# HUBioDataLab/DrugGEN

Hardware: AMD Instinct MI355X
Metric: molecules/sec GAN step (G+D fwd+bwd), N=45 graphs (higher is better)
Workload: dtype f32

## Files before the change

### druggen_amd/_lib.py

```python
from __future__ import annotations

import ctypes
import os
import threading
from ctypes import c_char_p, c_double, c_float, c_int, c_int64, c_size_t, c_void_p

import torch

_PKG = os.path.dirname(os.path.abspath(__file__))
LIB_PATH = os.environ.get("DG_LIB") or os.path.join(_PKG, "lib", "libdruggen_hip.so")

_P = c_void_p


class FFNFwdArgs(ctypes.Structure):
    _fields_ = [(n, _P) for n in ("x", "w1_packed", "b1", "w2_packed", "b2", "gamma", "beta", "y", "h", "relu_bits", "pre_ln",
                                  "mean", "rstd")] + [("R", c_int64), ("eps", c_float)]


class FFNBwdArgs(ctypes.Structure):
    _fields_ = [(n, _P) for n in ("x", "h", "relu_bits", "pre_ln", "mean", "rstd", "gamma", "w1_dgrad_packed", "w2_dgrad_packed",
                                  "dy", "dz_add", "dz", "dh", "dx", "dgamma", "dbeta", "dw1", "db1", "dw2", "db2", "workspace")] + [
        ("workspace_bytes", c_size_t), ("R", c_int64)]


SIGNATURES = {
    "dg_version": (c_int, []),
    "dg_last_error_string": (c_char_p, []),
    "dg_hidden_bytes": (c_size_t, [c_int64, c_int, c_int]),
    "dg_hidden_scale_offset": (c_size_t, [c_int64, c_int]),
    "dg_attn_core_fwd": (c_int, [_P] * 6 + [c_int, c_int, c_int, c_float, c_int, _P]),
    "dg_attn_core_bwd": (c_int, [_P] * 10 + [c_int, c_int, c_int, c_float, c_int, _P]),
    "dg_attn_core_bwd_add": (c_int, [_P] * 11 + [c_int, c_int, c_int, c_float, c_int, _P]),
    "dg_attn_core_bwd2": (c_int, [_P] * 16 + [c_int, c_int, c_int, c_float, c_int, _P]),
    "dg_attn_core_long_workspace_bytes": (c_size_t, [c_int, c_int, c_int]),
    "dg_attn_core_long_fwd": (c_int, [_P] * 6 + [c_int, c_int, c_int, c_float, c_int, _P]),
    "dg_attn_core_long_bwd": (c_int, [_P] * 12 + [c_size_t, c_int, c_int, c_int, c_float, c_int, _P]),
    "dg_attn_core_long_bwd2": (c_int, [_P] * 17 + [c_size_t, c_int, c_int, c_int, c_float, c_int, _P]),
    "dg_attn_half_packed_bytes": (c_size_t, [c_int]),
    "dg_attn_half_pack": (c_int, [_P, _P, _P, c_int, _P]),
    "dg_attn_half_fwd": (c_int, [_P] * 14 + [c_int, c_int, c_int, c_float, c_float, c_int, _P]),
    "dg_attn_half_f32_fwd": (c_int, [_P] * 17 + [c_int, c_int, c_int, c_float, c_float, _P]),
    "dg_attn_half_f32_bwd1_workspace_bytes": (c_size_t, [c_int]),
    "dg_attn_half_f32_bwd1": (c_int, [_P] * 19 + [_P, c_size_t, c_int, c_int, c_int, c_float, _P]),
    "dg_attn_half_bwd_workspace_bytes": (c_size_t, [c_int, c_int]),
    "dg_attn_half_bwd": (c_int, [_P] * 16 + [_P, c_size_t, c_int, c_int, c_int, c_float, c_int, _P]),
    "dg_ln_residual_fwd": (c_int, [_P] * 7 + [c_int64, c_int, c_float, c_int, _P]),
    "dg_ln_workspace_bytes": (c_size_t, [c_int64, c_int]),
    "dg_ln_residual_bwd": (c_int, [_P] * 9 + [_P, c_size_t, c_int64, c_int, c_int, _P]),
    "dg_ln_residual_bwd_add": (c_int, [_P] * 10 + [_P, c_size_t, c_int64, c_int, c_int, _P]),
    "dg_ln_residual_bwd2": (c_int, [_P] * 10 + [_P, c_size_t, c_int64, c_int, c_int, _P]),
    "dg_linear_wgrad_workspace_bytes": (c_size_t, [c_int64, c_int, c_int]),
    "dg_linear_wgrad": (c_int, [_P] * 5 + [_P, c_size_t, c_int64, c_int, c_int, c_int, _P]),
    "dg_row_gemm_packed_bytes": (c_size_t, [c_int, c_int, c_int]),
    "dg_row_gemm_pack": (c_int, [_P, _P, c_int, c_int, c_int, c_int, _P]),
    "dg_row_gemm_mask_words": (c_size_t, [c_int64, c_int, c_int, c_int]),
    "dg_row_gemm": (c_int, [_P] * 3 + [c_int64, c_int, c_int, _P, c_int, _P, _P, _P, _P, _P, _P, _P, _P, c_float, c_int, _P]),
    "dg_linear_wgrad3": (c_int, [_P] * 6 + [_P, c_size_t, c_int64, c_int, _P]),
    "dg_row_gemm_pack3": (c_int, [_P, _P, _P, _P, c_int, c_int, c_int, _P]),
    "dg_row_gemm_lin3": (c_int, [_P] * 5 + [c_int64, _P, _P, _P, c_int, _P]),
    "dg_row_gemm_sum3": (c_int, [_P] * 5 + [c_int64, _P, c_int, _P]),
    "dg_linear_wgrad_batch_begin": (c_int, []),
    "dg_linear_wgrad_batch_end": (c_int, [_P]),
    "dg_launch_pair_begin": (c_int, []),
    "dg_launch_pair_end": (c_int, [_P]),
    "dg_skinny_linear_fwd": (c_int, [_P] * 4 + [c_int64, c_int, c_int, c_int, _P]),
    "dg_skinny_linear_dgrad": (c_int, [_P] * 3 + [c_int64, c_int, c_int, c_int, _P]),
    "dg_skinny_linear_wgrad": (c_int, [_P] * 5 + [c_size_t, c_int64, c_int, c_int, c_int, _P]),
    "dg_embed_node_chain": (c_int, [_P] * 9 + [c_int64, c_int, c_int, _P]),
    "dg_embed_node_bwd": (c_int, [_P] * 8 + [c_int64, c_int, c_int, _P]),
    "dg_head_chain": (c_int, [_P] * 14 + [c_int64, c_int, _P]),
    "dg_head_bwd": (c_int, [_P] * 10 + [c_int64, c_int, _P]),
    "dg_head_wgrad": (c_int, [_P] * 12 + [c_int64, _P]),
    "dg_row_gemm_pack_batch": (c_int, [_P, c_int, c_int, c_int, _P]),
    "dg_row_gemm_ln_bwd_workspace_bytes": (c_size_t, [c_int]),
    "dg_row_gemm_ln_bwd": (c_int, [_P] * 3 + [c_int64, c_int] + [_P] * 7 + [_P, c_size_t, c_int, _P]),
    "dg_row_gemm_ln_bwd_in": (c_int, [_P] * 10 + [_P, c_size_t, c_int64, c_int, c_int, c_int, _P]),
    "dg_edge_ffn_ln_workspace_bytes": (c_size_t, [c_int64, c_int, c_int]),
    "dg_edge_ffn_ln_fwd": (c_int, [_P] * 13 + [c_int64, c_int, c_int, c_float, c_int, _P]),
    "dg_edge_ffn_ln_bwd": (c_int, [_P] * 20 + [_P, c_size_t, c_int64, c_int, c_int, c_int, _P]),
    "dg_edge_ffn_ln_fwd_pair": (c_int, [ctypes.POINTER(FFNFwdArgs), ctypes.POINTER(FFNFwdArgs), c_int, c_int, c_int, _P]),
    "dg_edge_ffn_ln_bwd_pair": (c_int, [ctypes.POINTER(FFNBwdArgs), ctypes.POINTER(FFNBwdArgs), c_int, c_int, c_int, _P]),
    "dg_ffn_f32_packed_bytes": (c_size_t, []),
    "dg_ffn_f32_pack": (c_int, [_P, _P, _P, _P]),
    "dg_ffn_ln_fwd_f32": (c_int, [ctypes.POINTER(FFNFwdArgs), ctypes.POINTER(FFNFwdArgs), _P]),
    "dg_ffn_bf16_padded_rows": (c_int64, [c_int64]),
    "dg_ffn_bf16_packed_bytes": (c_size_t, []),
    "dg_ffn_bf16_pack": (c_int, [_P, _P, _P, _P]),
    "dg_ffn_bf16_mask_words": (c_size_t, [c_int64]),
    "dg_ffn_bf16_workspace_bytes": (c_size_t, [c_int64]),
    "dg_ffn_ln_fwd_bf16": (c_int, [_P] * 11 + [c_int64, c_float, _P]),
    "dg_ffn_ln_bwd_bf16": (c_int, [_P] * 18 + [_P, c_size_t, c_int64, _P]),
    "dg_embed_sym_packed_floats": (c_size_t, []),
    "dg_embed_sym_workspace_bytes": (c_size_t, [c_int, c_int]),
    "dg_embed_sym_dgrad_packed_floats": (c_size_t, []),
    "dg_embed_sym_pack_dgrad": (c_int, [_P, _P, _P]),
    "dg_embed_sym_pack": (c_int, [_P, _P, _P]),
    "dg_embed_sym_fwd": (c_int, [_P] * 6 + [c_int] * 7 + [_P]),
    "dg_embed_sym_bwd": (c_int, [_P] * 12 + [_P, c_size_t] + [c_int] * 7 + [_P]),
    "dg_embed_sym_bwd_bf16_workspace_bytes": (c_size_t, [c_int, c_int]),
    "dg_embed_sym_bwd_bf16": (c_int, [_P] * 11 + [_P, c_size_t] + [c_int] * 6 + [_P]),
    "dg_embed_sym_bwd2": (c_int, [_P] * 11 + [_P, c_size_t] + [c_int] * 7 + [_P]),
    "dg_onehot_embed_workspace_bytes": (c_size_t, [c_int, c_int]),
    "dg_onehot_embed_fwd": (c_int, [_P, _P, _P, c_int, c_int, c_int, c_int, c_int, _P]),
    "dg_onehot_embed_bwd": (c_int, [_P, _P, _P, _P, c_size_t, c_int, c_int, c_int, c_int, c_int, _P]),
    "dg_densify": (c_int, [_P, _P, _P, c_int64, c_int, c_int, c_int, _P, _P, _P, _P]),
    "dg_mol_gather": (c_int, [_P, _P, _P, c_int64, _P, c_int, c_int, c_int, c_int, _P, _P, _P, _P, _P]),
    "dg_adamw_flat": (c_int, [_P, _P, _P, _P, c_int64, c_float, c_float, c_float, c_float, c_float, c_int64, _P]),
    "dg_adamw_flat_devstep": (c_int, [_P, _P, _P, _P, c_int64, c_float, c_float, c_float, c_float, c_float, _P, _P]),
    "dg_argmax_decode": (c_int, [_P, c_int64, c_int, _P, _P]),
    "dg_decode_graph": (c_int, [_P] * 3 + [c_int] * 5 + [_P] * 8 + [_P]),
    "dg_fp_pack": (c_int, [_P, c_int, c_int64, c_int, _P, _P, _P]),
    "dg_fp_tanimoto_workspace_bytes": (c_size_t, [c_int64, c_int64]),
    "dg_fp_tanimoto": (c_int, [_P, _P, c_int64, _P, _P, c_int64, c_int, c_int, _P, _P, _P, c_size_t, _P]),
    "dg_prof_enable": (c_int, [c_int]),
    "dg_prof_reset": (c_int, []),
    "dg_prof_read": (c_int, [c_int, ctypes.POINTER(c_int64), ctypes.POINTER(c_double)]),
    "dg_set_edge_rows": (c_int, [c_int64]),
    "dg_edge_rows": (c_int64, []),
}

KERNEL_IDS = {"attn_fwd": 0, "attn_bwd": 1, "attn_bwd2": 2, "ln_fwd": 3, "ln_bwd": 4, "ln_bwd2": 5, "linear_wgrad": 6, "row_gemm": 7, "embed_sym": 8, "ffn": 9, "ffn_wgrad": 10,
              "attn_half_fwd": 11, "attn_half_bwd": 12,
              "row_gemm_e128": 13, "row_gemm_e_n384": 14, "row_gemm_e_k384": 15,
              "linear_wgrad_e128": 16, "linear_wgrad_e_n384": 17, "linear_wgrad_e_k384": 18,
              "ffn_node": 19, "ffn_wgrad_node": 20, "ffn_f32": 21, "ffn_f32_node": 22}
EDGE_ROWS = 65536
_edge_rows = EDGE_ROWS


def edge_rows() -> int:
    return _edge_rows


def set_edge_rows(rows: int = 0) -> None:
# ... 104 lines not shown
```

### druggen_amd/functional/attention.py

```python
from __future__ import annotations

import contextlib
import ctypes
import threading

import torch
from torch.autograd import Function
from torch.autograd.function import once_differentiable

from .. import _lib
from ..options import options
from ._runtime import *
from .layernorm import *
from .dense import *
from .heads import *
from .ffn import *


def _attn_shapes(q, e):
    B, N, C = q.shape
    if tuple(e.shape) != (B, N, N, C):
        raise RuntimeError(f"attn_core: edge tensor {tuple(e.shape)} does not match node tensor {tuple(q.shape)}")
    return B, N, C

# ... 96 lines not shown
    @staticmethod
    def forward(ctx, q, k, v, e, ws, wo, alpha):
        B, N, C = _attn_shapes(q, e)
        ws = None if ws is None else _c(ws)
        wo = _c(wo)
        dq, dk, dv = torch.empty_like(q), torch.empty_like(q), torch.empty_like(q)
        de = torch.empty_like(e)
        _core_bwd(q, k, v, e, ws, wo, None, dq, dk, dv, de, alpha)
        ctx.save_for_backward(q, k, v, e, ws, wo)
        ctx.alpha = alpha
        return dq, dk, dv, de

    @staticmethod
    @once_differentiable
    def backward(ctx, tq, tk, tv, te):
        q, k, v, e, ws, wo = ctx.saved_tensors
        B, N, C = _attn_shapes(q, e)
        tq, tk, tv, te = _c(tq), _c(tk), _c(tv), _c(te)
        gq, gk, gv = torch.empty_like(q), torch.empty_like(q), torch.empty_like(q)
        ge = torch.empty_like(e)
        gws = torch.empty_like(e) if ws is not None else None
        gwo = torch.empty_like(q)
        _core_bwd2(q, k, v, e, ws, wo, tq, tk, tv, te, gq, gk, gv, ge, gws, gwo, ctx.alpha)
        return gq, gk, gv, ge, gws, gwo, None


def attn_core(q, k, v, e, alpha: float, need_s: bool = True):
    s, o = _AttnCore.apply(q, k, v, e, float(alpha), bool(need_s))
    return (s if need_s else None), o


def _composite_attn_block(x1, y, wq, bq, wk, bk, wv, bv, we, be, woe, boe, won, bon, g3, b3, g4, b4, alpha, eps3,
                          eps4, need_edge):
    q, k, v = linear(x1, wq, bq), linear(x1, wk, bk), linear(x1, wv, bv)
    e = linear(y, we, be)
    s, o = attn_core(q, k, v, e, alpha, need_s=need_edge)
    x2 = linear_ln(o, won, bon, x1, g3, b3, eps3)
    if not need_edge:
        return x2
    return x2, linear_ln(s, woe, boe, y, g4, b4, eps4)


def attn_half_f32_supported(yf, N: int, C: int) -> bool:
    mode = options.attn_half_f32
    return yf.is_cuda and yf.dtype == torch.float32 and C == 128 and N <= (48 if mode == "n48" else 96) and mode != "off"


def attn_half_f32_bwd1_supported(dy2f, B: int, N: int, C: int, graph: bool = False) -> bool:
    mode = options.attn_half_f32_bwd
    return (dy2f.is_cuda and dy2f.dtype == torch.float32 and C == 128 and N <= 48 and mode != "off"
            and (B >= 128 or mode == "force") and (not graph or mode != "nograph"))


class _AttnBlock(Function):

    @staticmethod
    def forward(ctx, x1, y, wq, bq, wk, bk, wv, bv, we, be, woe, boe, won, bon, g3, b3, g4, b4, alpha, eps3, eps4,
                need_edge, ppre=None, pmean=None, prstd=None, pgamma=None, pbeta=None):
        B, N, C = x1.shape
        _check_neighbours(N)
        x1f, yf = _c(x1).reshape(-1, C), _c(y).reshape(-1, C)
        adt = x1f.dtype
        pw = lambda w_, m_: packed_weight(w_, m_, adt)
        if lin3_supported(x1f, (wq, wk, wv)):
            q, k, v = lin3(x1f, (wq, wk, wv), (bq, bk, bv))
        else:
            q = row_gemm(x1f, pw(wq, 0), C, C, bias=bq)
            k = row_gemm(x1f, pw(wk, 0), C, C, bias=bk)
            v = row_gemm(x1f, pw(wv, 0), C, C, bias=bv)
        lib = _lib.load()
        keep = any(ctx.needs_input_grad)
        o = torch.empty_like(q)
        fused_edge = need_edge and attn_half_f32_supported(yf, N, C)
        if fused_edge:
            R = yf.shape[0]
            dev = yf.device
            e = torch.empty(R, C, dtype=adt, device=dev) if keep else None
            s = torch.empty(R, C, dtype=adt, device=dev) if keep else None
            y2 = torch.empty(R, C, dtype=adt, device=dev)
            pre4 = torch.empty(R, C, dtype=adt, device=dev) if keep else None
            mean4 = torch.empty(R, dtype=torch.float32, device=dev)
            rstd4 = torch.empty(R, dtype=torch.float32, device=dev)
            with _dev(q):
                _lib.check(lib.dg_attn_half_f32_fwd(_lib.ptr(yf), _lib.ptr(q), _lib.ptr(k), _lib.ptr(v), pw(we, 0).data_ptr(),
                                                    _lib.fptr(_c(be)), pw(woe, 0).data_ptr(), _lib.fptr(_c(boe)), _lib.fptr(_c(g4)),
                                                    _lib.fptr(_c(b4)), _lib.ptr(e), _lib.ptr(s), _lib.ptr(o), _lib.ptr(y2),
                                                    _lib.ptr(pre4), _lib.ptr(mean4), _lib.ptr(rstd4), B, N, C, alpha, eps4,
                                                    _lib.stream_of(q)), "dg_attn_half_f32_fwd")
            _account("attn_half_fwd", 4 * (R * C * (5 if keep else 2) + 4 * B * N * C), 4 * R * C * C,
                     floor=4 * (R * C * 2 + 4 * B * N * C))
        else:
            e = row_gemm(yf, pw(we, 0), C, C, bias=be)
            s = torch.empty_like(e) if need_edge else None
            _core_fwd(q, k, v, e, s, o, alpha, B, N, C)
        r3 = row_gemm(o, pw(won, 0), C, C, bias=bon, residual=x1f, ln=(_c(g3), _c(b3), eps3), want_pre=keep)
        x2, mean3, rstd3, pre3 = r3 if keep else (*r3, None)
        outs = [x2.view(B, N, C)]
        ctx.alias = bool(keep and in_second_order_forward() and _alias_outputs_enabled())
        aliases = ()
        if ctx.alias:
            aliases = tuple(_weight_alias(t) for t in (wq, wk, wv, we, woe, won, g3, g4))
            wq, wk, wv, we, woe, won, g3, g4 = aliases
        saved = [x1, y, wq, wk, wv, we, woe, won, g3, g4, q, k, v, e, s, o, mean3, rstd3, pre3]
        if need_edge:
            if not fused_edge:
                r4 = row_gemm(s, pw(woe, 0), C, C, bias=boe, residual=yf, ln=(_c(g4), _c(b4), eps4), want_pre=keep)
                y2, mean4, rstd4, pre4 = r4 if keep else (*r4, None)
            outs.append(y2.view(B, N, N, C))
            saved += [mean4, rstd4, pre4]
        else:
            pre4 = None
        ctx.has_prev = ppre is not None
        if ctx.has_prev:
            saved += [ppre, pmean, prstd, pgamma]
        ctx.save_for_backward(*saved)
        ctx.cfg = (alpha, eps3, eps4, need_edge, (B, N, C))
        ctx.extra = (bq, bk, bv, be, boe, bon, b3, b4)
        ctx.set_materialize_grads(False)
        return tuple(outs) + ((pre3, pre4) if need_edge else (pre3,)) + (q, k, v, e) + aliases

    @staticmethod
    def backward(ctx, dx2, *more):
        alpha, eps3, eps4, need_edge, (B, N, C) = ctx.cfg
        galias = ()
        if ctx.alias:
            more, galias = more[:-8], more[-8:]
        sv = ctx.saved_tensors
        x1, y, wq, wk, wv, we, woe, won, g3, g4, q, k, v, e, s, o, mean3, rstd3, pre3 = sv[:19]
        mean4, rstd4, pre4 = sv[19:22] if need_edge else (None, None, None)
        bq, bk, bv, be, boe, bon, b3, b4 = ctx.extra
        if need_edge:
            dy2, add3, add4, aq, ak, av, ae = more
            if dy2 is None:
                dy2 = torch.zeros_like(pre4)
        else:
            dy2 = add4 = None
            add3, aq, ak, av, ae = more
        if dx2 is None:
            dx2 = torch.zeros_like(pre3)
        wants_w = ctx.needs_input_grad[2] and not _inputs_only()
        want_aff = any(ctx.needs_input_grad[14:18]) and not _inputs_only()
        ppre = pmean = prstd = pgamma = None
        if ctx.has_prev:
            ppre, pmean, prstd, pgamma = sv[-4:]
        second_pass = any(t is not None for t in (add3, add4, aq, ak, av, ae))
        fuse_prev = bool(ctx.has_prev and not torch.is_grad_enabled() and not second_pass and ctx.needs_input_grad[1]
                         and ctx.needs_input_grad[22] and row_gemm_ln_bwd_supported(q, C)
                         and tuple(ppre.shape) == (B * N * N, C))
        outs = _AttnBlockBwd.apply(x1, y, wq, bq, wk, bk, wv, bv, we, be, woe, boe, won, bon, g3, g4,
                                   q, k, v, e, s, o, mean3, rstd3, pre3, mean4, rstd4, pre4, dx2, dy2,
                                   add3, add4, aq, ak, av, ae,
                                   alpha, need_edge, ctx.needs_input_grad[0], ctx.needs_input_grad[1], wants_w,
                                   ppre if fuse_prev else None, pmean, prstd, pgamma, want_aff,
                                   not torch.is_grad_enabled())
        (dx1, dy, dwq, dbq, dwk, dbk, dwv, dbv, dwe, dbe, dwoe, dboe, dwon, dbon, dg3, db3, dg4, db4, dzp, dgp, dbp) = outs
        if any(g is not None for g in galias):
            dwq, dwk, dwv, dwe, dwoe, dwon, dg3, dg4 = _join_alias_grads((dwq, dwk, dwv, dwe, dwoe, dwon, dg3, dg4), galias)
        if not (ctx.needs_input_grad[25] and not _inputs_only()):
            dgp = dbp = None
        return (dx1, dy, dwq, dbq, dwk, dbk, dwv, dbv, dwe, dbe, dwoe, dboe, dwon, dbon, dg3, db3, dg4, db4,
                None, None, None, None, dzp, None, None, dgp, dbp)


def _attn_bwd_launch(q, k, v, e, ws, wo, alpha, add_e=None):
    dq, dk, dv = torch.empty_like(q), torch.empty_like(q), torch.empty_like(q)
    de = torch.empty_like(e)
    _core_bwd(q, k, v, e, ws, wo, add_e, dq, dk, dv, de, alpha)
    return dq, dk, dv, de


def _attn_bwd2_launch(q, k, v, e, ws, wo, tq, tk, tv, te, alpha):
    gq, gk, gv, gwo = (torch.empty_like(q) for _ in range(4))
    ge = torch.empty_like(e)
    gws = torch.empty_like(e) if ws is not None else None
    _core_bwd2(q, k, v, e, ws, wo, tq, tk, tv, te, gq, gk, gv, ge, gws, gwo, alpha)
    return gq, gk, gv, ge, gws, gwo


class _AttnBlockBwd(Function):

    @staticmethod
    def forward(ctx, *args):
        wants_w = args[40] or (len(args) > 45 and args[45])
        with _reduce_batch(args[0], on=bool(wants_w)) as inb:
            return _AttnBlockBwd._forward(ctx, inb, *args)

    @staticmethod
    def _forward(ctx, inb, x1, y, wq, bq, wk, bk, wv, bv, we, be, woe, boe, won, bon, g3, g4, q, k, v, e, s, o,
                 mean3, rstd3, pre3, mean4, rstd4, pre4, dx2, dy2, add3, add4, aq, ak, av, ae,
                 alpha, need_edge, want_x, want_y, wants_w, ppre=None, pmean=None, prstd=None, pgamma=None, want_aff=None,
                 no_graph=False):
        if want_aff is None:
            want_aff = wants_w
        B, N, C = x1.shape
        adt = q.dtype
        pw = lambda w_, m_: packed_weight(w_, m_, adt)
        cast = lambda t: t if t.dtype == adt else t.to(adt)
        x1f, yf = _c(x1).reshape(-1, C), _c(y).reshape(-1, C)
        dx2f = _c(cast(dx2)).reshape(-1, C)
        cadd = lambda t: None if t is None else _c(cast(t)).reshape(-1, C)
        dz3, dg3, db3 = _ln_bwd_rows(pre3, g3, mean3, rstd3, dx2f, cadd(add3), want_affine=want_aff,
                                     batch_slot=0 if inb else None)
# ... 297 lines not shown
```

### druggen_amd/options.py

```python
from __future__ import annotations

import contextlib
import os

_CHOICES = {
    "hidden": ("dh16", "dh24", "f32", "f24", "f16"),
    "ffn_f32": ("unfused", "fused"),
    "attn_half_f32": ("fused", "n48", "off"),
    "attn_half_f32_bwd": ("fused", "nograph", "off", "force"),
    "attn_half": ("fused", "unfused", "force"),
    "ffn_bf16": ("fused", "unfused"),
    "low_memory_share": ("auto", "on", "off"),
    "ln_bwd_epilogue": (True, False),
    "ln_bwd_prologue": (True, False),
    "ffn_pair": (True, False),
    "penalty_wgrad": ("joined", "engine"),
    "embed_bf16": ("fast", "general"),
}
_ENV = {"hidden": "DG_HIDDEN", "ffn_f32": "DG_FFN_F32", "attn_half_f32": "DG_ATTN_HALF_F32",
        "attn_half_f32_bwd": "DG_ATTN_HALF_F32_BWD", "attn_half": "DG_ATTN_HALF", "ffn_bf16": "DG_FFN_BF16",
        "low_memory_share": "DG_LOW_MEMORY_SHARE"}


class _Options:
    def __init__(self):
        for name, choices in _CHOICES.items():
            value = choices[0]
            env = _ENV.get(name)
            if env and os.environ.get(env) is not None:
                value = os.environ[env]
                if value not in choices:
                    raise ValueError(f"{env}={value!r}: expected one of {choices}")
            object.__setattr__(self, name, value)

    def __setattr__(self, name, value):
        if name not in _CHOICES:
            raise AttributeError(f"druggen_amd.options has no option {name!r}")
        if value not in _CHOICES[name]:
            raise ValueError(f"options.{name} = {value!r}: expected one of {_CHOICES[name]}")
        object.__setattr__(self, name, value)

    def set(self, **kw):
        for k, v in kw.items():
            setattr(self, k, v)

    @contextlib.contextmanager
    def override(self, **kw):
        prev = {k: getattr(self, k) for k in kw}
        self.set(**kw)
        try:
            yield self
        finally:
            self.set(**prev)

    def as_dict(self):
        return {k: getattr(self, k) for k in _CHOICES}


options = _Options()
```

### include/druggen_hip.h

```cpp
#ifndef DRUGGEN_HIP_H
#define DRUGGEN_HIP_H

#include <stddef.h>
#include <stdint.h>

#ifdef __cplusplus
extern "C" {
#endif

#define DG_VERSION 232
#define DG_DTYPE_F32  0
#define DG_DTYPE_BF16 1
#define DG_DTYPE_F32_H16 2
#define DG_DTYPE_F32_H24 3
#define DG_DTYPE_F32_DH16 4
#define DG_DTYPE_F32_DH24 5
#define DG_DTYPE_F32_H32 6
#define DG_DTYPE_F32_H32_DH16 7
#define DG_E_SHAPE   (-1)
#define DG_E_ARG     (-2)
#define DG_E_WORKSPACE (-3)
#define DG_EDGE_ROWS 65536

typedef void* dg_stream_t;
// ... 99 lines not shown
int dg_row_gemm_pack_batch(const void* table, int n, int max_dim, int dtype, dg_stream_t stream);
int dg_row_gemm_pack3(const float* w0, const float* w1, const float* w2, void* packed, int cols, int mode, int dtype,
                      dg_stream_t stream);
int dg_row_gemm_lin3(const void* a, const void* packed, void* y0, void* y1, void* y2, int64_t R, const float* b0,
                     const float* b1, const float* b2, int dtype, dg_stream_t stream);
int dg_row_gemm_sum3(const void* a0, const void* a1, const void* a2, const void* packed, void* y, int64_t R,
                     const void* residual, int dtype, dg_stream_t stream);
size_t dg_row_gemm_mask_words(int64_t R, int K, int N, int dtype);
int dg_row_gemm(const void* a, const void* packed, void* y, int64_t R, int K, int N,
                const float* bias, int relu, unsigned* relu_bits_out, const unsigned* mask_bits,
                const void* residual,
                const float* gamma, const float* beta, float* mean, float* rstd, void* pre_ln,
                float eps, int dtype, dg_stream_t stream);
size_t dg_row_gemm_ln_bwd_workspace_bytes(int dtype);
int dg_row_gemm_ln_bwd(const void* a, const void* packed, void* dz, int64_t R, int K, const void* residual,
                       const void* ln_pre, const float* ln_mean, const float* ln_rstd, const float* ln_gamma,
                       float* dgamma, float* dbeta, void* workspace, size_t workspace_bytes, int dtype,
                       dg_stream_t stream);
int dg_row_gemm_ln_bwd_in(const void* dy, const void* ln_pre, const float* ln_mean, const float* ln_rstd,
                          const float* ln_gamma, const void* packed, void* dz, void* y, float* dgamma, float* dbeta,
                          void* workspace, size_t workspace_bytes, int64_t R, int K, int N, int dtype,
                          dg_stream_t stream);

size_t dg_edge_ffn_ln_workspace_bytes(int64_t R, int C, int H);
int dg_edge_ffn_ln_fwd(const void* x, const void* w1_packed, const float* b1, const void* w2_packed,
                       const float* b2, const float* gamma, const float* beta,
                       void* y, void* h, unsigned* relu_bits, void* pre_ln, float* mean, float* rstd,
                       int64_t R, int C, int H, float eps, int dtype, dg_stream_t stream);
int dg_edge_ffn_ln_bwd(const void* x, const void* h, const unsigned* relu_bits, const void* pre_ln,
                       const float* mean, const float* rstd, const float* gamma,
                       const void* w1_dgrad_packed, const void* w2_dgrad_packed, const void* dy,
                       const void* dz_add,
                       void* dz, void* dh, void* dx, float* dgamma, float* dbeta,
                       float* dw1, float* db1, float* dw2, float* db2,
                       void* workspace, size_t workspace_bytes, int64_t R, int C, int H, int dtype,
                       dg_stream_t stream);

typedef struct dg_ffn_fwd_args {
    const void* x; const void* w1_packed; const float* b1; const void* w2_packed; const float* b2;
    const float* gamma; const float* beta;
    void* y; void* h; unsigned* relu_bits; void* pre_ln; float* mean; float* rstd;
    int64_t R; float eps;
} dg_ffn_fwd_args;
typedef struct dg_ffn_bwd_args {
    const void* x; const void* h; const unsigned* relu_bits; const void* pre_ln; const float* mean; const float* rstd;
    const float* gamma; const void* w1_dgrad_packed; const void* w2_dgrad_packed; const void* dy; const void* dz_add;
    void* dz; void* dh; void* dx; float* dgamma; float* dbeta; float* dw1; float* db1; float* dw2; float* db2;
    void* workspace; size_t workspace_bytes; int64_t R;
} dg_ffn_bwd_args;
int dg_edge_ffn_ln_fwd_pair(const dg_ffn_fwd_args* node, const dg_ffn_fwd_args* edge, int C, int H, int dtype,
                            dg_stream_t stream);
int dg_edge_ffn_ln_bwd_pair(const dg_ffn_bwd_args* node, const dg_ffn_bwd_args* edge, int C, int H, int dtype,
                            dg_stream_t stream);

int64_t dg_ffn_bf16_padded_rows(int64_t R);
size_t dg_ffn_bf16_packed_bytes(void);
int dg_ffn_bf16_pack(const float* w1, const float* w2, void* packed, dg_stream_t stream);
size_t dg_ffn_bf16_mask_words(int64_t R);
size_t dg_ffn_bf16_workspace_bytes(int64_t R);
int dg_ffn_ln_fwd_bf16(const void* x, const void* packed, const float* b1, const float* b2, const float* gamma,
                       const float* beta, void* y, void* pre_ln, float* mean, float* rstd, unsigned* relu_bits,
                       int64_t R, float eps, dg_stream_t stream);
int dg_ffn_ln_bwd_bf16(const void* x, const void* pre_ln, const float* mean, const float* rstd,
                       const unsigned* relu_bits, const float* gamma, const void* packed, const float* b1,
                       const void* dy, void* dz, void* dx, float* dgamma, float* dbeta,
                       float* dw1, float* db1, float* dw2, float* db2, unsigned* bits_scratch,
                       void* workspace, size_t workspace_bytes, int64_t R, dg_stream_t stream);


size_t dg_ffn_f32_packed_bytes(void);
int dg_ffn_f32_pack(const float* w1, const float* w2, void* packed, dg_stream_t stream);
int dg_ffn_ln_fwd_f32(const dg_ffn_fwd_args* node, const dg_ffn_fwd_args* edge, dg_stream_t stream);

size_t dg_embed_sym_packed_floats(void);
size_t dg_embed_sym_workspace_bytes(int B, int N);
int dg_embed_sym_pack(const float* w2, float* packed, dg_stream_t stream);
size_t dg_embed_sym_dgrad_packed_floats(void);
int dg_embed_sym_pack_dgrad(const float* w2, float* packed, dg_stream_t stream);
int dg_embed_sym_fwd(const float* a, const float* w1, const float* b1, const float* w2_packed, const float* b2,
                     void* out, int B, int N, int E, int H, int C, int act, int dtype, dg_stream_t stream);
int dg_embed_sym_bwd(const float* a, const float* w1, const float* b1, const float* w2_packed,
                     const float* w2_dgrad_packed, const float* b2, const void* g,
                     float* da, float* dw1, float* db1, float* dw2, float* db2,
                     void* workspace, size_t workspace_bytes,
                     int B, int N, int E, int H, int C, int act, int dtype, dg_stream_t stream);
size_t dg_embed_sym_bwd_bf16_workspace_bytes(int B, int N);
int dg_embed_sym_bwd_bf16(const float* a, const float* w1, const float* b1, const float* w2, const float* b2,
                          const void* g, float* da, float* dw1, float* db1, float* dw2, float* db2,
                          void* workspace, size_t workspace_bytes, int B, int N, int E, int H, int C, int act,
                          dg_stream_t stream);

int dg_embed_sym_bwd2(const float* a, const float* w1, const float* b1, const float* w2_packed,
                      const float* w2_dgrad_packed, const float* b2, const void* g, const float* t,
                      void* gg, float* gw1, float* gw2, void* workspace, size_t workspace_bytes,
                      int B, int N, int E, int H, int C, int act, int dtype, dg_stream_t stream);

size_t dg_onehot_embed_workspace_bytes(int E, int C);
int dg_onehot_embed_fwd(const int* labels, const float* table, void* out, int B, int N, int E, int C, int dtype,
                        dg_stream_t stream);
int dg_onehot_embed_bwd(const int* labels, const void* g, float* dtable, void* workspace, size_t workspace_bytes,
                        int B, int N, int E, int C, int dtype, dg_stream_t stream);

int dg_densify(const int64_t* edge_src, const int64_t* edge_dst, const int64_t* edge_attr, int64_t n_edges,
               int B, int N, int E, int* labels, float* a, int* bad_count, dg_stream_t stream);

int dg_mol_gather(const uint8_t* atoms, const int64_t* ptr, const uint32_t* entries, int64_t n, const int64_t* index, int B,
// ... 84 lines not shown
```

Measured before the change: 4862.

## Run attention block forward and backward as single native sequenced entry points

Adds dg_attn_block_fwd/bwd C entry points that issue the whole attention block's kernel sequence (qkv projection, edge projection and attention, output projections with LayerNorm, and the full backward including weight gradients) from one ctypes call. It also carves all intermediate buffers from a single allocation and bypasses the nested autograd backward Function. The aim is to cut Python dispatch, per-op ctypes overhead and allocator calls in a launch-bound small-graph workload. It is enabled by default through a new option, at the cost of a second code path that must stay consistent with the existing one.

```diff
diff --git a/druggen_amd/_lib.py b/druggen_amd/_lib.py
--- a/druggen_amd/_lib.py
+++ b/druggen_amd/_lib.py
@@ -3,7 +3,7 @@
 import ctypes
 import os
 import threading
-from ctypes import c_char_p, c_double, c_float, c_int, c_int64, c_size_t, c_void_p
+from ctypes import c_char_p, c_double, c_float, c_int, c_int64, c_size_t, c_uint, c_void_p
 
 import torch
 
@@ -22,6 +22,25 @@
     _fields_ = [(n, _P) for n in ("x", "h", "relu_bits", "pre_ln", "mean", "rstd", "gamma", "w1_dgrad_packed", "w2_dgrad_packed",
                                   "dy", "dz_add", "dz", "dh", "dx", "dgamma", "dbeta", "dw1", "db1", "dw2", "db2", "workspace")] + [
         ("workspace_bytes", c_size_t), ("R", c_int64)]
+
+
+class AttnBlockFwdArgs(ctypes.Structure):
+    _fields_ = [(n, _P) for n in ("x1", "y", "wqkv_packed", "bq", "bk", "bv", "we_packed", "be", "woe_packed", "boe", "won_packed",
+                                  "bon", "g3", "b3", "g4", "b4", "q", "k", "v", "o", "e", "s", "x2", "mean3", "rstd3", "pre3",
+                                  "y2", "mean4", "rstd4", "pre4")] + [
+        ("B", c_int), ("N", c_int), ("C", c_int), ("alpha", c_float), ("eps3", c_float), ("eps4", c_float), ("flags", c_uint)]
+
+
+class AttnBlockBwdArgs(ctypes.Structure):
+    _fields_ = [(n, _P) for n in ("x1", "y", "q", "k", "v", "e", "s", "o", "mean3", "rstd3", "pre3", "mean4", "rstd4", "pre4", "g3",
+                                  "g4", "won_dgrad_packed", "woe_dgrad_packed", "we_dgrad_packed", "wqkv_dgrad_packed", "dx2",
+                                  "dy2", "ppre", "pmean", "prstd", "pgamma", "dz3", "d_o", "dz4", "ds", "de", "dq", "dk", "dv",
+                                  "dx1", "dy", "dzp", "dgp", "dbp", "dg3", "db3", "dg4", "db4", "dwqkv", "dbqkv", "dwe", "dbe",
+                                  "dwon", "dbon", "dwoe", "dboe", "workspace")] + [
+        ("workspace_bytes", c_size_t), ("B", c_int), ("N", c_int), ("C", c_int), ("alpha", c_float), ("flags", c_uint)]
+
+
+AB_NEED_EDGE, AB_WGRAD, AB_AFFINE, AB_INPUTS_ONLY, AB_REDUCE_BATCH, AB_BWD1_FUSED, AB_LN4_IN_GEMM = 1, 2, 4, 8, 16, 32, 64
 
 
 SIGNATURES = {
@@ -81,6 +100,9 @@
     "dg_edge_ffn_ln_bwd": (c_int, [_P] * 20 + [_P, c_size_t, c_int64, c_int, c_int, c_int, _P]),
     "dg_edge_ffn_ln_fwd_pair": (c_int, [ctypes.POINTER(FFNFwdArgs), ctypes.POINTER(FFNFwdArgs), c_int, c_int, c_int, _P]),
     "dg_edge_ffn_ln_bwd_pair": (c_int, [ctypes.POINTER(FFNBwdArgs), ctypes.POINTER(FFNBwdArgs), c_int, c_int, c_int, _P]),
+    "dg_attn_block_workspace_bytes": (c_size_t, [c_int, c_int, c_int, c_uint]),
+    "dg_attn_block_fwd": (c_int, [ctypes.POINTER(AttnBlockFwdArgs), _P]),
+    "dg_attn_block_bwd": (c_int, [ctypes.POINTER(AttnBlockBwdArgs), _P]),
     "dg_ffn_f32_packed_bytes": (c_size_t, []),
     "dg_ffn_f32_pack": (c_int, [_P, _P, _P, _P]),
     "dg_ffn_ln_fwd_f32": (c_int, [ctypes.POINTER(FFNFwdArgs), ctypes.POINTER(FFNFwdArgs), _P]),
diff --git a/druggen_amd/csrc/attn_block_seq.hip b/druggen_amd/csrc/attn_block_seq.hip
--- /dev/null
+++ b/druggen_amd/csrc/attn_block_seq.hip
@@ -0,0 +1,162 @@
+#include "common.h"
+
+using namespace dg;
+
+namespace {
+
+constexpr size_t align256(size_t n) { return (n + 255) / 256 * 256; }
+
+struct BwdLayout {
+    size_t ln3, ln4, lnp, w3, we, won, woe;
+    size_t total() const { return ln3 + ln4 + lnp + w3 + we + won + woe; }
+};
+
+BwdLayout bwd_layout(int B, int N, int C) {
+    const int64_t RN = static_cast<int64_t>(B) * N, RE = RN * N;
+    BwdLayout l{};
+    l.ln3 = align256(dg_ln_workspace_bytes(RN, C));
+    size_t ln4 = dg_ln_workspace_bytes(RE, C);
+    const size_t half = dg_attn_half_f32_bwd1_workspace_bytes(B), gemm = dg_row_gemm_ln_bwd_workspace_bytes(DG_DTYPE_F32);
+    ln4 = ln4 > half ? ln4 : half;
+    ln4 = ln4 > gemm ? ln4 : gemm;
+    l.ln4 = align256(ln4);
+    l.lnp = align256(gemm);
+    l.w3 = align256(dg_linear_wgrad_workspace_bytes(RN, 3 * C, C));
+    l.we = align256(dg_linear_wgrad_workspace_bytes(RE, C, C));
+    l.won = align256(dg_linear_wgrad_workspace_bytes(RN, C, C));
+    l.woe = l.we;
+    return l;
+}
+
+int shape_check(const char* who, int B, int N, int C) {
+    if (B < 1 || N < 1 || N > 96 || C != 128)
+        return fail(DG_E_SHAPE, "%s: needs dim 128 and 1..96 neighbours (got B=%d N=%d C=%d)", who, B, N, C);
+    return 0;
+}
+
+}
+
+extern "C" size_t dg_attn_block_workspace_bytes(int B, int N, int C, unsigned flags) {
+    (void)flags;
+    if (B < 1 || N < 1 || N > 96 || C != 128) return 0;
+    return bwd_layout(B, N, C).total();
+}
+
+extern "C" int dg_attn_block_fwd(const dg_attn_block_fwd_args* a, dg_stream_t stream) {
+    if (!a) return fail(DG_E_ARG, "dg_attn_block_fwd: null argument block");
+    if (int st = shape_check("dg_attn_block_fwd", a->B, a->N, a->C)) return st;
+    const bool need_edge = a->flags & DG_ATTN_BLOCK_NEED_EDGE;
+    if (!a->x1 || !a->y || !a->wqkv_packed || !a->we_packed || !a->won_packed || !a->be || !a->bon || !a->g3 || !a->b3 ||
+        !a->q || !a->k || !a->v || !a->o || !a->x2 || !a->mean3 || !a->rstd3)
+        return fail(DG_E_ARG, "dg_attn_block_fwd: null pointer");
+    if (need_edge ? (!a->woe_packed || !a->boe || !a->g4 || !a->b4 || !a->y2 || !a->mean4 || !a->rstd4) : !a->e)
+        return fail(DG_E_ARG, "dg_attn_block_fwd: null pointer (edge side)");
+    const int B = a->B, N = a->N, C = a->C;
+    const int64_t RN = static_cast<int64_t>(B) * N, RE = RN * N;
+    int st = dg_row_gemm_lin3(a->x1, a->wqkv_packed, a->q, a->k, a->v, RN, a->bq, a->bk, a->bv, DG_DTYPE_F32, stream);
+    if (st) return st;
+    if (need_edge) {
+        st = dg_attn_half_f32_fwd(a->y, a->q, a->k, a->v, a->we_packed, a->be, a->woe_packed, a->boe, a->g4, a->b4, a->e, a->s,
+                                  a->o, a->y2, a->pre4, a->mean4, a->rstd4, B, N, C, a->alpha, a->eps4, stream);
+    } else {
+        st = dg_row_gemm(a->y, a->we_packed, a->e, RE, C, C, a->be, 0, nullptr, nullptr, nullptr, nullptr, nullptr, nullptr,
+                         nullptr, nullptr, 0.f, DG_DTYPE_F32, stream);
+        if (!st) st = dg_attn_core_fwd(a->q, a->k, a->v, a->e, nullptr, a->o, B, N, C, a->alpha, DG_DTYPE_F32, stream);
+    }
+    if (st) return st;
+    return dg_row_gemm(a->o, a->won_packed, a->x2, RN, C, C, a->bon, 0, nullptr, nullptr, a->x1, a->g3, a->b3, a->mean3,
+                       a->rstd3, a->pre3, a->eps3, DG_DTYPE_F32, stream);
+}
+
+extern "C" int dg_attn_block_bwd(const dg_attn_block_bwd_args* a, dg_stream_t stream) {
+    if (!a) return fail(DG_E_ARG, "dg_attn_block_bwd: null argument block");
+    if (int st = shape_check("dg_attn_block_bwd", a->B, a->N, a->C)) return st;
+    const unsigned f = a->flags;
+    const bool need_edge = f & DG_ATTN_BLOCK_NEED_EDGE, inputs_only = f & DG_ATTN_BLOCK_INPUTS_ONLY;
+    const bool wants_w = (f & DG_ATTN_BLOCK_WGRAD) && !inputs_only, want_aff = (f & DG_ATTN_BLOCK_AFFINE) && !inputs_only;
+    const bool batch = f & DG_ATTN_BLOCK_REDUCE_BATCH;
+    const bool fused1 = need_edge && (f & DG_ATTN_BLOCK_BWD1_FUSED), ln4_in = need_edge && !fused1 && (f & DG_ATTN_BLOCK_LN4_IN_GEMM);
+    const int B = a->B, N = a->N, C = a->C;
+    const int64_t RN = static_cast<int64_t>(B) * N, RE = RN * N;
+    if (!a->x1 || !a->y || !a->q || !a->k || !a->v || !a->e || !a->o || !a->mean3 || !a->rstd3 || !a->pre3 || !a->g3 ||
+        !a->won_dgrad_packed || !a->dx2 || !a->dz3 || !a->d_o || !a->de || !a->dq || !a->dk || !a->dv || !a->workspace)
+        return fail(DG_E_ARG, "dg_attn_block_bwd: null pointer");
+    if (need_edge && (!a->s || !a->mean4 || !a->rstd4 || !a->pre4 || !a->g4 || !a->woe_dgrad_packed || !a->dy2 || !a->dz4 ||
+                      (!fused1 && !a->ds)))
+        return fail(DG_E_ARG, "dg_attn_block_bwd: null pointer (edge side)");
+    if ((wants_w || want_aff) && !batch)
+        return fail(DG_E_ARG, "dg_attn_block_bwd: parameter gradients need DG_ATTN_BLOCK_REDUCE_BATCH (their workspaces are read at its end)");
+    if (fused1 && N > 48) return fail(DG_E_SHAPE, "dg_attn_block_bwd: DG_ATTN_BLOCK_BWD1_FUSED serves at most 48 neighbours (got %d)", N);
+    if (want_aff && (!a->dg3 || a->db3 != a->dg3 + C || (need_edge && (!a->dg4 || a->db4 != a->dg4 + C))))
+        return fail(DG_E_ARG, "dg_attn_block_bwd: dgamma / dbeta of a LayerNorm must be adjacent ([2,C])");
+    if (wants_w && (!a->dwqkv || !a->dwe || !a->dwon || (need_edge && !a->dwoe)))
+        return fail(DG_E_ARG, "dg_attn_block_bwd: null weight gradient");
+    if ((a->dy || a->dzp) && !a->we_dgrad_packed) return fail(DG_E_ARG, "dg_attn_block_bwd: dy needs the e projection's input-gradient pack");
+    if (a->dzp && (!a->ppre || !a->pmean || !a->prstd || !a->pgamma))
+        return fail(DG_E_ARG, "dg_attn_block_bwd: dzp needs the producing LayerNorm's saved tensors");
+    if (a->dx1 && !a->wqkv_dgrad_packed) return fail(DG_E_ARG, "dg_attn_block_bwd: dx1 needs the q / k / v input-gradient pack");
+    const BwdLayout l = bwd_layout(B, N, C);
+    if (a->workspace_bytes < l.total()) return fail(DG_E_WORKSPACE, "dg_attn_block_bwd: workspace too small");
+    char* ws3 = static_cast<char*>(a->workspace);
+    char* ws4 = ws3 + l.ln3;
+    char* wsp = ws4 + l.ln4;
+    char* wsw = wsp + l.lnp;
+
+    if (batch) dg_linear_wgrad_batch_begin();
+    const auto done = [&](int st) {
+        if (!batch) return st;
+        const int st2 = dg_linear_wgrad_batch_end(stream);
+        return st ? st : st2;
+    };
+    float* const dg3 = want_aff ? a->dg3 : nullptr;
+    float* const dg4 = want_aff && need_edge ? a->dg4 : nullptr;
+    int st = dg_ln_residual_bwd_add(a->pre3, nullptr, a->g3, a->mean3, a->rstd3, a->dx2, nullptr, a->dz3, dg3, dg3 ? dg3 + C : nullptr,
+                                    ws3, l.ln3, RN, C, DG_DTYPE_F32, stream);
+    if (!st)
+        st = dg_row_gemm(a->dz3, a->won_dgrad_packed, a->d_o, RN, C, C, nullptr, 0, nullptr, nullptr, nullptr, nullptr, nullptr,
+                         nullptr, nullptr, nullptr, 0.f, DG_DTYPE_F32, stream);
+    if (st) return done(st);
+    if (fused1) {
+        st = dg_attn_half_f32_bwd1(a->dy2, a->pre4, a->mean4, a->rstd4, a->g4, a->woe_dgrad_packed, a->e, a->q, a->k, a->v, a->d_o,
+                                   a->dz4, nullptr, a->de, a->dq, a->dk, a->dv, dg4, dg4 ? dg4 + C : nullptr, ws4, l.ln4, B, N, C,
+                                   a->alpha, stream);
+    } else {
+        if (ln4_in) {
+            st = dg_row_gemm_ln_bwd_in(a->dy2, a->pre4, a->mean4, a->rstd4, a->g4, a->woe_dgrad_packed, a->dz4, a->ds, dg4,
+                                       dg4 ? dg4 + C : nullptr, ws4, l.ln4, RE, C, C, DG_DTYPE_F32, stream);
+        } else if (need_edge) {
+            st = dg_ln_residual_bwd_add(a->pre4, nullptr, a->g4, a->mean4, a->rstd4, a->dy2, nullptr, a->dz4, dg4,
+                                        dg4 ? dg4 + C : nullptr, ws4, l.ln4, RE, C, DG_DTYPE_F32, stream);
+            if (!st)
+                st = dg_row_gemm(a->dz4, a->woe_dgrad_packed, a->ds, RE, C, C, nullptr, 0, nullptr, nullptr, nullptr, nullptr,
+                                 nullptr, nullptr, nullptr, nullptr, 0.f, DG_DTYPE_F32, stream);
+        }
+        if (!st)
+            st = dg_attn_core_bwd_add(a->q, a->k, a->v, a->e, need_edge ? a->ds : nullptr, a->d_o, nullptr, a->dq, a->dk, a->dv,
+                                      a->de, B, N, C, a->alpha, DG_DTYPE_F32, stream);
+    }
+    if (st) return done(st);
+    const float* dz4 = need_edge ? a->dz4 : nullptr;
+    if (a->dzp)
+        st = dg_row_gemm_ln_bwd(a->de, a->we_dgrad_packed, a->dzp, RE, C, dz4, a->ppre, a->pmean, a->prstd, a->pgamma, a->dgp, a->dbp,
+                                wsp, l.lnp, DG_DTYPE_F32, stream);
+    else if (a->dy)
+        st = dg_row_gemm(a->de, a->we_dgrad_packed, a->dy, RE, C, C, nullptr, 0, nullptr, nullptr, dz4, nullptr, nullptr, nullptr,
+                         nullptr, nullptr, 0.f, DG_DTYPE_F32, stream);
+    if (!st && a->dx1)
+        st = dg_row_gemm_sum3(a->dq, a->dk, a->dv, a->wqkv_dgrad_packed, a->dx1, RN, a->dz3, DG_DTYPE_F32, stream);
+    if (st || !wants_w) return done(st);
+    st = dg_linear_wgrad3(a->dq, a->dk, a->dv, a->x1, a->dwqkv, a->dbqkv, wsw, l.w3, RN, DG_DTYPE_F32, stream);
+    if (!st) st = dg_linear_wgrad(a->de, nullptr, a->y, a->dwe, a->dbe, wsw + l.w3, l.we, RE, C, C, DG_DTYPE_F32, stream);
+    if (st) return done(st);
+    if (need_edge) dg_launch_pair_begin();
+    st = dg_linear_wgrad(a->dz3, nullptr, a->o, a->dwon, a->dbon, wsw + l.w3 + l.we, l.won, RN, C, C, DG_DTYPE_F32, stream);
+    if (need_edge) {
+        if (!st)
+            st = dg_linear_wgrad(a->dz4, nullptr, a->s, a->dwoe, a->dboe, wsw + l.w3 + l.we + l.won, l.woe, RE, C, C, DG_DTYPE_F32,
+                                 stream);
+        const int st2 = dg_launch_pair_end(stream);
+        st = st ? st : st2;
+    }
+    return done(st);
+}
diff --git a/druggen_amd/functional/attention.py b/druggen_amd/functional/attention.py
--- a/druggen_amd/functional/attention.py
+++ b/druggen_amd/functional/attention.py
@@ -172,6 +172,160 @@
             and (B >= 128 or mode == "force") and (not graph or mode != "nograph"))
 
 
+attn_block_seq_calls = [0, 0]
+_seq_ws_need = {}
+
+
+def _attn_block_seq_static(x1, y, N, C, mats, vecs) -> bool:
+    return (x1.is_cuda and x1.dtype == torch.float32 and y.dtype == torch.float32 and C == 128 and 1 <= N <= ATTN_SHORT_MAX_N
+            and x1.shape[0] >= 1 and tuple(y.shape[-3:]) == (N, N, C)
+            and all(w.dtype == torch.float32 and tuple(w.shape) == (128, 128) for w in mats)
+            and all(b is not None and b.dtype == torch.float32 and tuple(b.shape) == (128,) for b in vecs))
+
+
+def _carve(dev, *floats):
+    offs, total = [], 0
+    for n in floats:
+        offs.append(total)
+        total += (n + 63) // 64 * 64
+    flat = torch.empty(total, dtype=torch.float32, device=dev)
+    return [flat[o:o + n] if n else None for o, n in zip(offs, floats)]
+
+
+def _dp(t):
+    return None if t is None else t.data_ptr()
+
+
+def _seq_account_fwd(B, N, C, keep, need_edge):
+    RN, RE = B * N, B * N * N
+    _account(_gemm_key(RN, 128, 384), 4 * RN * (128 + 384), 2 * RN * 128 * 384)
+    if need_edge:
+        _account("attn_half_fwd", 4 * (RE * C * (5 if keep else 2) + 4 * B * N * C), 4 * RE * C * C,
+                 floor=4 * (RE * C * 2 + 4 * B * N * C))
+    else:
+        _account(_gemm_key(RE, C, C), RE * 8 * C, 2 * RE * C * C)
+        _account("attn_fwd", 4 * B * (N * N * C + 4 * N * C))
+    _account(_gemm_key(RN, C, C), RN * 4 * C * (3 + keep), 2 * RN * C * C, floor=RN * 12 * C)
+
+
+def _seq_account_bwd(B, N, C, need_edge, fused1, ln4_in, prev, want_y, want_x, wants_w):
+    RN, RE = B * N, B * N * N
+    _account("ln_bwd", 4 * RN * C * 3)
+    _account(_gemm_key(RN, C, C), RN * 8 * C, 2 * RN * C * C)
+    if fused1:
+        _account("attn_half_bwd", 4 * (RE * C * 5 + 7 * B * N * C), 2 * RE * C * C)
+    else:
+        if ln4_in:
+            _account(_gemm_key(RE, 128, 128), 4 * RE * 128 * 4, 2 * RE * 128 * 128)
+        elif need_edge:
+            _account("ln_bwd", 4 * RE * C * 3)
+            _account(_gemm_key(RE, C, C), RE * 8 * C, 2 * RE * C * C)
+        base = 4 * B * ((3 if need_edge else 2) * N * N * C + 7 * N * C)
+        _account("attn_bwd", base, floor=base)
+    if prev:
+        _account(_gemm_key(RE, C, 128), 4 * RE * (C + 128 * (3 if need_edge else 2)), 2 * RE * C * 128)
+    elif want_y:
+        _account(_gemm_key(RE, C, C), RE * 4 * C * (3 if need_edge else 2), 2 * RE * C * C)
+    if want_x:
+        _account(_gemm_key(RN, 384, 128), 4 * RN * (384 + 128 * 2), 2 * RN * 384 * 128)
+    if wants_w:
+        _account(_wgrad_key(RN, 384, 128), 4 * RN * (384 + 128), 2 * RN * 384 * 128)
+        _account(_wgrad_key(RE, C, C), 8 * RE * C, 2 * RE * C * C)
+        _account(_wgrad_key(RN, C, C), 8 * RN * C, 2 * RN * C * C)
+        if need_edge:
+            _account(_wgrad_key(RE, C, C), 8 * RE * C, 2 * RE * C * C)
+
+
+def _attn_block_seq_fwd(x1f, yf, wq, bq, wk, bk, wv, bv, we, be, woe, boe, won, bon, g3, b3, g4, b4, alpha, eps3, eps4, need_edge,
+                        keep, B, N, C):
+    dev = x1f.device
+    RN, RE = B * N, B * N * N
+    nc, ec = RN * C, RE * C
+    edge_kept = ec if (keep or not need_edge) else 0
+    q, k, v, o, mean3, rstd3, pre3, e, s, mean4, rstd4, pre4 = _carve(
+        dev, nc, nc, nc, nc, RN, RN, nc if keep else 0, edge_kept, ec if (keep and need_edge) else 0,
+        RE if need_edge else 0, RE if need_edge else 0, ec if (keep and need_edge) else 0)
+    x2 = torch.empty(RN, C, dtype=torch.float32, device=dev)
+    y2 = torch.empty(RE, C, dtype=torch.float32, device=dev) if need_edge else None
+    g3, b3, g4, b4 = _c(g3), _c(b3), _c(g4), _c(b4)
+    bq, bk, bv, be, boe, bon = _c(bq), _c(bk), _c(bv), _c(be), _c(boe), _c(bon)
+    a = _lib.AttnBlockFwdArgs(
+        x1f.data_ptr(), yf.data_ptr(), packed_weight3(wq, wk, wv, 0).data_ptr(), bq.data_ptr(), bk.data_ptr(), bv.data_ptr(),
+        packed_weight(we, 0).data_ptr(), be.data_ptr(), packed_weight(woe, 0).data_ptr() if need_edge else None, boe.data_ptr(),
+        packed_weight(won, 0).data_ptr(), bon.data_ptr(), g3.data_ptr(), b3.data_ptr(), g4.data_ptr(), b4.data_ptr(),
+        q.data_ptr(), k.data_ptr(), v.data_ptr(), o.data_ptr(), _dp(e), _dp(s), x2.data_ptr(), mean3.data_ptr(), rstd3.data_ptr(),
+        _dp(pre3), _dp(y2), _dp(mean4), _dp(rstd4), _dp(pre4), B, N, C, alpha, eps3, eps4, _lib.AB_NEED_EDGE if need_edge else 0)
+    with _dev(x1f):
+        _lib.check(_lib.load().dg_attn_block_fwd(ctypes.byref(a), _lib.stream_of(x1f)), "dg_attn_block_fwd")
+    attn_block_seq_calls[0] += 1
+    _seq_account_fwd(B, N, C, keep, need_edge)
+    m = lambda t, rows: None if t is None else t.view(rows, C)
+    return (m(q, RN), m(k, RN), m(v, RN), m(e, RE), m(s, RE), m(o, RN), x2, mean3, rstd3, m(pre3, RN), y2, mean4, rstd4,
+            m(pre4, RE))
+
+
+def _attn_block_seq_bwd(sv, dx2, dy2, alpha, need_edge, B, N, C, want_x, want_y, wants_w, want_aff, prev):
+    x1, y, wq, wk, wv, we, woe, won, g3, g4, q, k, v, e, s, o, mean3, rstd3, pre3 = sv[:19]
+    mean4, rstd4, pre4 = sv[19:22] if need_edge else (None, None, None)
+    dev = q.device
+    RN, RE = B * N, B * N * N
+    nc, ec = RN * C, RE * C
+    x1f, yf = _c(x1).reshape(-1, C), _c(y).reshape(-1, C)
+    dx2f = _c(dx2).reshape(-1, C)
+    dy2f = _c(dy2).reshape(-1, C) if need_edge else None
+    fused1 = need_edge and attn_half_f32_bwd1_supported(dy2f, B, N, C, graph=False)
+    ln4_in = need_edge and not fused1 and RE >= _lib.edge_rows() and ln_bwd_row_gemm_supported(dy2f, C, C)
+    batch = wants_w or want_aff
+    flags = ((_lib.AB_NEED_EDGE if need_edge else 0) | (_lib.AB_WGRAD if wants_w else 0) | (_lib.AB_AFFINE if want_aff else 0)
+             | (_lib.AB_INPUTS_ONLY if _inputs_only() else 0) | (_lib.AB_REDUCE_BATCH if batch else 0)
+             | (_lib.AB_BWD1_FUSED if fused1 else 0) | (_lib.AB_LN4_IN_GEMM if ln4_in else 0))
+    dz3, do, dq, dk, dv, de, dz4, ds = _carve(dev, nc, nc, nc, nc, nc, ec, ec if need_edge else 0,
+                                              ec if (need_edge and not fused1) else 0)
+    aff, eaff = (C if want_aff else 0), (C if want_aff and need_edge else 0)
+    w, ew = (C * C if wants_w else 0), (C * C if wants_w and need_edge else 0)
+    bw, ebw = (C if wants_w else 0), (C if wants_w and need_edge else 0)
+    pb = C if prev is not None else 0
+    dg3, db3, dg4, db4, dgp, dbp, dw3, db3w, dwe, dbe, dwon, dbon, dwoe, dboe = _carve(
+        dev, aff, aff, eaff, eaff, pb, pb, 3 * w, 3 * bw, w, bw, w, bw, ew, ebw)
+    dx1 = torch.empty(RN, C, dtype=torch.float32, device=dev) if want_x else None
+    dy = dzp = None
+    if prev is not None:
+        dzp = torch.empty(RE, C, dtype=torch.float32, device=dev)
+    elif want_y:
+        dy = torch.empty(RE, C, dtype=torch.float32, device=dev)
+    g3c, g4c = _c(g3), _c(g4)
+    pgc = _c(prev[3]) if prev is not None else None
+    lib = _lib.load()
+    need = _seq_ws_need.get((B, N))
+    if need is None:
+        need = _seq_ws_need[(B, N)] = int(lib.dg_attn_block_workspace_bytes(B, N, C, 0))
+    with _dev(q):
+        ws = _scratch(q, need, "attn_block")
+        a = _lib.AttnBlockBwdArgs(
+            x1f.data_ptr(), yf.data_ptr(), q.data_ptr(), k.data_ptr(), v.data_ptr(), e.data_ptr(), _dp(s), o.data_ptr(),
+            mean3.data_ptr(), rstd3.data_ptr(), pre3.data_ptr(), _dp(mean4), _dp(rstd4), _dp(pre4), g3c.data_ptr(), g4c.data_ptr(),
+            packed_weight(won, 1).data_ptr(), packed_weight(woe, 1).data_ptr() if need_edge else None,
+            packed_weight(we, 1).data_ptr() if (want_y or prev is not None) else None,
+            packed_weight3(wq, wk, wv, 1).data_ptr() if want_x else None,
+            dx2f.data_ptr(), _dp(dy2f), *((_dp(prev[0]), _dp(prev[1]), _dp(prev[2]), _dp(pgc)) if prev is not None else (None,) * 4),
+            dz3.data_ptr(), do.data_ptr(), _dp(dz4), _dp(ds), de.data_ptr(), dq.data_ptr(), dk.data_ptr(), dv.data_ptr(),
+            _dp(dx1), _dp(dy), _dp(dzp), _dp(dgp), _dp(dbp), _dp(dg3), _dp(db3), _dp(dg4), _dp(db4),
+            _dp(dw3), _dp(db3w), _dp(dwe), _dp(dbe), _dp(dwon), _dp(dbon), _dp(dwoe), _dp(dboe),
+            ws.data_ptr(), ws.numel(), B, N, C, alpha, flags)
+        _lib.check(lib.dg_attn_block_bwd(ctypes.byref(a), _lib.stream_of(q)), "dg_attn_block_bwd")
+    attn_block_seq_calls[1] += 1
+    _seq_account_bwd(B, N, C, need_edge, fused1, ln4_in, prev is not None, want_y, want_x, wants_w)
+    gw = [None] * 12
+    if wants_w:
+        w3, b3 = dw3.view(384, 128), db3w
+        gw[0:6] = [w3[0:128], b3[0:128], w3[128:256], b3[128:256], w3[256:384], b3[256:384]]
+        gw[6], gw[7], gw[10], gw[11] = dwe.view(C, C), dbe, dwon.view(C, C), dbon
+        if need_edge:
+            gw[8], gw[9] = dwoe.view(C, C), dboe
+    return (None if dx1 is None else dx1.view(x1.shape), None if dy is None else dy.view(y.shape), *gw, dg3, db3, dg4, db4,
+            dzp, dgp, dbp)
+
+
 class _AttnBlock(Function):
 
     @staticmethod
@@ -182,6 +336,18 @@
         x1f, yf = _c(x1).reshape(-1, C), _c(y).reshape(-1, C)
         adt = x1f.dtype
         pw = lambda w_, m_: packed_weight(w_, m_, adt)
+        keep = any(ctx.needs_input_grad)
+        ctx.seq_ok = _attn_block_seq_static(x1, y, N, C, (wq, wk, wv, we, woe, won), (bq, bk, bv, be, boe, bon, g3, b3, g4, b4))
+        seq = (ctx.seq_ok and options.attn_block_seq and not in_second_order_forward()
+               and (not need_edge or attn_half_f32_supported(yf, N, C)))
+        fused_edge = need_edge and attn_half_f32_supported(yf, N, C)
+        if seq:
+            (q, k, v, e, s, o, x2, mean3, rstd3, pre3, y2, mean4, rstd4, pre4) = _attn_block_seq_fwd(
+                x1f, yf, wq, bq, wk, bk, wv, bv, we, be, woe, boe, won, bon, g3, b3, g4, b4, alpha, eps3, eps4, need_edge, keep,
+                B, N, C)
+            return _AttnBlock._finish_forward(ctx, x1, y, wq, bq, wk, bk, wv, bv, we, be, woe, boe, won, bon, g3, b3, g4, b4,
+                                              alpha, eps3, eps4, need_edge, ppre, pmean, prstd, pgamma, keep, B, N, C, q, k, v, e,
+                                              s, o, x2, mean3, rstd3, pre3, y2, mean4, rstd4, pre4)
         if lin3_supported(x1f, (wq, wk, wv)):
             q, k, v = lin3(x1f, (wq, wk, wv), (bq, bk, bv))
         else:
@@ -189,9 +355,7 @@
             k = row_gemm(x1f, pw(wk, 0), C, C, bias=bk)
             v = row_gemm(x1f, pw(wv, 0), C, C, bias=bv)
         lib = _lib.load()
-        keep = any(ctx.needs_input_grad)
         o = torch.empty_like(q)
-        fused_edge = need_edge and attn_half_f32_supported(yf, N, C)
         if fused_edge:
             R = yf.shape[0]
             dev = yf.device
@@ -215,6 +379,19 @@
             _core_fwd(q, k, v, e, s, o, alpha, B, N, C)
         r3 = row_gemm(o, pw(won, 0), C, C, bias=bon, residual=x1f, ln=(_c(g3), _c(b3), eps3), want_pre=keep)
         x2, mean3, rstd3, pre3 = r3 if keep else (*r3, None)
+        if not need_edge:
+            y2 = mean4 = rstd4 = pre4 = None
+        elif not fused_edge:
+            r4 = row_gemm(s, pw(woe, 0), C, C, bias=boe, residual=yf, ln=(_c(g4), _c(b4), eps4), want_pre=keep)
+            y2, mean4, rstd4, pre4 = r4 if keep else (*r4, None)
+        return _AttnBlock._finish_forward(ctx, x1, y, wq, bq, wk, bk, wv, bv, we, be, woe, boe, won, bon, g3, b3, g4, b4,
+                                          alpha, eps3, eps4, need_edge, ppre, pmean, prstd, pgamma, keep, B, N, C, q, k, v, e,
+                                          s, o, x2, mean3, rstd3, pre3, y2, mean4, rstd4, pre4)
+
+    @staticmethod
+    def _finish_forward(ctx, x1, y, wq, bq, wk, bk, wv, bv, we, be, woe, boe, won, bon, g3, b3, g4, b4, alpha, eps3, eps4,
+                        need_edge, ppre, pmean, prstd, pgamma, keep, B, N, C, q, k, v, e, s, o, x2, mean3, rstd3, pre3, y2,
+                        mean4, rstd4, pre4):
         outs = [x2.view(B, N, C)]
         ctx.alias = bool(keep and in_second_order_forward() and _alias_outputs_enabled())
         aliases = ()
@@ -223,9 +400,6 @@
             wq, wk, wv, we, woe, won, g3, g4 = aliases
         saved = [x1, y, wq, wk, wv, we, woe, won, g3, g4, q, k, v, e, s, o, mean3, rstd3, pre3]
         if need_edge:
-            if not fused_edge:
-                r4 = row_gemm(s, pw(woe, 0), C, C, bias=boe, residual=yf, ln=(_c(g4), _c(b4), eps4), want_pre=keep)
-                y2, mean4, rstd4, pre4 = r4 if keep else (*r4, None)
             outs.append(y2.view(B, N, N, C))
             saved += [mean4, rstd4, pre4]
         else:
@@ -267,7 +441,13 @@
         fuse_prev = bool(ctx.has_prev and not torch.is_grad_enabled() and not second_pass and ctx.needs_input_grad[1]
                          and ctx.needs_input_grad[22] and row_gemm_ln_bwd_supported(q, C)
                          and tuple(ppre.shape) == (B * N * N, C))
-        outs = _AttnBlockBwd.apply(x1, y, wq, bq, wk, bk, wv, bv, we, be, woe, boe, won, bon, g3, g4,
+        if (ctx.seq_ok and options.attn_block_seq and not torch.is_grad_enabled() and not second_pass and not ctx.alias
+                and dx2.dtype == torch.float32 and (dy2 is None or dy2.dtype == torch.float32)
+                and (not fuse_prev or (ppre.dtype == torch.float32 and pgamma.dtype == torch.float32))):
+            outs = _attn_block_seq_bwd(sv, dx2, dy2, alpha, need_edge, B, N, C, ctx.needs_input_grad[0], ctx.needs_input_grad[1],
+                                       wants_w, want_aff, (ppre, pmean, prstd, pgamma) if fuse_prev else None)
+        else:
+            outs = _AttnBlockBwd.apply(x1, y, wq, bq, wk, bk, wv, bv, we, be, woe, boe, won, bon, g3, g4,
                                    q, k, v, e, s, o, mean3, rstd3, pre3, mean4, rstd4, pre4, dx2, dy2,
                                    add3, add4, aq, ak, av, ae,
                                    alpha, need_edge, ctx.needs_input_grad[0], ctx.needs_input_grad[1], wants_w,
diff --git a/druggen_amd/options.py b/druggen_amd/options.py
--- a/druggen_amd/options.py
+++ b/druggen_amd/options.py
@@ -13,6 +13,7 @@
     "low_memory_share": ("auto", "on", "off"),
     "ln_bwd_epilogue": (True, False),
     "ln_bwd_prologue": (True, False),
+    "attn_block_seq": (True, False),
     "ffn_pair": (True, False),
     "penalty_wgrad": ("joined", "engine"),
     "embed_bf16": ("fast", "general"),
diff --git a/include/druggen_hip.h b/include/druggen_hip.h
--- a/include/druggen_hip.h
+++ b/include/druggen_hip.h
@@ -175,6 +175,42 @@
                             dg_stream_t stream);
 int dg_edge_ffn_ln_bwd_pair(const dg_ffn_bwd_args* node, const dg_ffn_bwd_args* edge, int C, int H, int dtype,
                             dg_stream_t stream);
+
+#define DG_ATTN_BLOCK_NEED_EDGE    1u
+#define DG_ATTN_BLOCK_WGRAD        2u
+#define DG_ATTN_BLOCK_AFFINE       4u
+#define DG_ATTN_BLOCK_INPUTS_ONLY  8u
+#define DG_ATTN_BLOCK_REDUCE_BATCH 16u
+#define DG_ATTN_BLOCK_BWD1_FUSED   32u
+#define DG_ATTN_BLOCK_LN4_IN_GEMM  64u
+typedef struct dg_attn_block_fwd_args {
+    const float* x1; const float* y;
+    const void* wqkv_packed; const float* bq; const float* bk; const float* bv;
+    const void* we_packed; const float* be; const void* woe_packed; const float* boe;
+    const void* won_packed; const float* bon;
+    const float* g3; const float* b3; const float* g4; const float* b4;
+    float* q; float* k; float* v; float* o; float* e; float* s;
+    float* x2; float* mean3; float* rstd3; float* pre3;
+    float* y2; float* mean4; float* rstd4; float* pre4;
+    int B; int N; int C; float alpha; float eps3; float eps4; unsigned flags;
+} dg_attn_block_fwd_args;
+typedef struct dg_attn_block_bwd_args {
+    const float* x1; const float* y; const float* q; const float* k; const float* v; const float* e; const float* s;
+    const float* o; const float* mean3; const float* rstd3; const float* pre3; const float* mean4; const float* rstd4;
+    const float* pre4; const float* g3; const float* g4;
+    const void* won_dgrad_packed; const void* woe_dgrad_packed; const void* we_dgrad_packed; const void* wqkv_dgrad_packed;
+    const float* dx2; const float* dy2;
+    const float* ppre; const float* pmean; const float* prstd; const float* pgamma;
+    float* dz3; float* d_o; float* dz4; float* ds; float* de; float* dq; float* dk; float* dv;
+    float* dx1; float* dy; float* dzp; float* dgp; float* dbp;
+    float* dg3; float* db3; float* dg4; float* db4;
+    float* dwqkv; float* dbqkv; float* dwe; float* dbe; float* dwon; float* dbon; float* dwoe; float* dboe;
+    void* workspace; size_t workspace_bytes;
+    int B; int N; int C; float alpha; unsigned flags;
+} dg_attn_block_bwd_args;
+size_t dg_attn_block_workspace_bytes(int B, int N, int C, unsigned flags);
+int dg_attn_block_fwd(const dg_attn_block_fwd_args* args, dg_stream_t stream);
+int dg_attn_block_bwd(const dg_attn_block_bwd_args* args, dg_stream_t stream);
 
 int64_t dg_ffn_bf16_padded_rows(int64_t R);
 size_t dg_ffn_bf16_packed_bytes(void);
```

New measurement: 4862, median of 2. About the same (-0.0%).
